# quantumgizmos/ldpc

Measured on AMD Instinct MI355X. Metric: syndromes_per_sec_batched_bp50_product_sum_ldpc36_n10k, higher is better.
Workload: dtype f64; 1 GPU; configs[1]: (3,6)-regular LDPC n=10000 (m=5000, E=30000), product_sum flooding BP, max_iter=50, batch=65536 syndromes per GPU, BSC p=0.09, code seed 1, error seed 7; batch_per_gpu=65536, global_batch=65536, max_iter=50, outputs=decoding u8, log_prob_ratios f64, iterations i32, converge u8, parallelism=single GPU, no process group, device_math=libm_exact

## Files before the change

### include/ldpc_hip.h

```cpp
#ifndef LDPC_HIP_H
#define LDPC_HIP_H

#include <stdint.h>

#ifdef __cplusplus
extern "C" {
#endif

typedef enum {
    LDPC_HIP_OK = 0,
    LDPC_HIP_ERR_INVALID = -1,
    LDPC_HIP_ERR_DEVICE = -2,
    LDPC_HIP_ERR_NOMEM = -3,
    LDPC_HIP_ERR_UNSUPPORTED = -4
} ldpc_hip_status;

#define LDPC_HIP_PRODUCT_SUM 0
#define LDPC_HIP_MINIMUM_SUM 1

typedef struct {
    int32_t m;
    int32_t n;
    int32_t nnz;
    const int32_t *csr_row_ptr;
// ... 79 lines not shown
int ldpc_hip_bp_last_phase_ms(ldpc_hip_bp *h, float *persistent_ms, float *per_pass_ms);

int64_t ldpc_hip_bp_workspace_bytes(const ldpc_hip_bp *h, int64_t batch);

int ldpc_hip_bp_set_tuning(ldpc_hip_bp *h, int32_t waves_per_workgroup, int32_t max_chunk_tiles);

int ldpc_hip_bp_set_ring(ldpc_hip_bp *h, int32_t depth);

int ldpc_hip_bp_set_handoff(ldpc_hip_bp *h, int32_t threshold_tiles);

int ldpc_hip_bp_set_small_code_kernel(ldpc_hip_bp *h, int32_t mode);
int ldpc_hip_bp_set_debug_switch(ldpc_hip_bp *h, const char *name, int32_t value);

#define LDPC_HIP_MATH_LIBM_EXACT 0
#define LDPC_HIP_MATH_FAST 1
int ldpc_hip_bp_set_math(ldpc_hip_bp *h, int32_t math_mode);

int ldpc_hip_bp_clock_probe(ldpc_hip_bp *h, uint64_t *cycles, uint64_t *ticks, double *tick_hz);

int ldpc_hip_bp_copy_probe(ldpc_hip_bp *h, int64_t tiles, int32_t segments_per_tile, int32_t passes, float *ms, double *gbytes_per_s);

int64_t ldpc_hip_debug_device_buf_bytes(void);

void *ldpc_hip_host_alloc(size_t bytes);
void ldpc_hip_host_free(void *p);

const char *ldpc_hip_last_error(void);
const char *ldpc_hip_version(void);

typedef struct ldpc_hip_bp_multi ldpc_hip_bp_multi;
int ldpc_hip_bp_multi_create(const ldpc_hip_bp_desc *desc , const int32_t *device_ids,
                             int32_t ndev, ldpc_hip_bp_multi **out);
void ldpc_hip_bp_multi_destroy(ldpc_hip_bp_multi *mh);
int32_t ldpc_hip_bp_multi_devices(const ldpc_hip_bp_multi *mh);
ldpc_hip_bp *ldpc_hip_bp_multi_handle(ldpc_hip_bp_multi *mh, int32_t i);
int ldpc_hip_bp_multi_decode_batch(ldpc_hip_bp_multi *mh, int32_t with_osd, const uint8_t *syndromes, int64_t batch,
                                   uint8_t *decoding, double *llr, int32_t *iterations, uint8_t *converge);
int ldpc_hip_bp_multi_last_kernel_ms(ldpc_hip_bp_multi *mh, float *ms_per_device);
int ldpc_hip_bp_multi_set_staging(ldpc_hip_bp_multi *mh, int32_t force);

#ifdef __cplusplus
}
#endif
#endif
```

### ldpc_amd/_lib.py

```python
from __future__ import annotations

import ctypes as C
import os

_HERE = os.path.dirname(os.path.abspath(__file__))
LIB_PATH = os.environ.get("LDPC_HIP_LIB") or os.path.join(_HERE, "lib", "libldpc_hip.so")

SYMBOLS = (
    "ldpc_hip_bp_create", "ldpc_hip_bp_destroy", "ldpc_hip_bp_set_channel", "ldpc_hip_bp_set_params",
    "ldpc_hip_bp_set_stream", "ldpc_hip_bp_set_schedule", "ldpc_hip_bp_set_random_serial", "ldpc_hip_bp_get_schedule_order", "ldpc_hip_bp_decode_batch", "ldpc_hip_bp_decode_batch_async", "ldpc_hip_bposd0_decode_batch", "ldpc_hip_bposd0_decode_batch_async",
    "ldpc_hip_bp_set_osd", "ldpc_hip_bposd_get_status", "ldpc_hip_bp_set_osd_kernel", "ldpc_hip_bp_set_repack", "ldpc_hip_bp_set_serial_kernel", "ldpc_hip_bposd_decode_batch", "ldpc_hip_bposd_decode_batch_async",
    "ldpc_hip_bp_set_observables", "ldpc_hip_bp_decode_b8", "ldpc_hip_bp_soft_info_decode_batch", "ldpc_hip_pack_b8", "ldpc_hip_unpack_b8", "ldpc_hip_bp_last_phase_ms", "ldpc_hip_bp_clock_probe", "ldpc_hip_bp_copy_probe", "ldpc_hip_debug_device_buf_bytes", "ldpc_hip_host_alloc", "ldpc_hip_host_free",
    "ldpc_hip_gf2_mulvec_batch", "ldpc_hip_gen_bsc_syndromes", "ldpc_hip_bp_last_kernel_ms",
    "ldpc_hip_bp_workspace_bytes", "ldpc_hip_bp_set_tuning", "ldpc_hip_bp_set_math", "ldpc_hip_bp_set_ring", "ldpc_hip_bp_set_small_code_kernel", "ldpc_hip_bp_set_handoff", "ldpc_hip_last_error", "ldpc_hip_version",
    "ldpc_hip_bp_set_debug_switch", "ldpc_hip_bp_multi_create", "ldpc_hip_bp_multi_destroy", "ldpc_hip_bp_multi_devices", "ldpc_hip_bp_multi_handle",
    "ldpc_hip_bp_multi_decode_batch", "ldpc_hip_bp_multi_last_kernel_ms", "ldpc_hip_bp_multi_set_staging",
    "ldpc_hip_bp_decode_batch_priors", "ldpc_hip_bp_decode_batch_priors_async", "ldpc_hip_bposd0_decode_batch_priors", "ldpc_hip_bposd0_decode_batch_priors_async",
)


class BpDesc(C.Structure):
    _fields_ = [
        ("m", C.c_int32), ("n", C.c_int32), ("nnz", C.c_int32),
        ("csr_row_ptr", C.POINTER(C.c_int32)), ("csr_col_idx", C.POINTER(C.c_int32)),
        ("channel_probs", C.POINTER(C.c_double)),
        ("max_iter", C.c_int32), ("bp_method", C.c_int32),
        ("ms_scaling_factor", C.c_double), ("device", C.c_int32),
    ]


class LdpcHipError(RuntimeError):
    pass


_lib = None
# ... 32 lines not shown
            getattr(lib, name).argtypes = [vp, vp, i64, vp, vp, vp, vp, vp]
    lib.ldpc_hip_bp_set_osd.argtypes = [vp, i32, i32]
    lib.ldpc_hip_bposd_get_status.argtypes = [vp, vp, i64]
    lib.ldpc_hip_bp_set_osd_kernel.argtypes = [vp, i32]
    lib.ldpc_hip_bp_set_repack.argtypes = [vp, i32]
    lib.ldpc_hip_bp_set_serial_kernel.argtypes = [vp, i32]
    lib.ldpc_hip_bp_set_observables.argtypes = [vp, i32, vp, vp]
    lib.ldpc_hip_bp_decode_b8.argtypes = [vp, vp, i64, i32, vp, vp, vp, vp]
    lib.ldpc_hip_pack_b8.argtypes = [vp, vp, i64, i32, vp]
    lib.ldpc_hip_unpack_b8.argtypes = [vp, vp, i64, i32, vp]
    lib.ldpc_hip_bp_soft_info_decode_batch.argtypes = [vp, vp, i64, C.c_double, C.c_double, vp, vp, vp, vp, vp]
    lib.ldpc_hip_bposd_decode_batch.argtypes = [vp, vp, i64, vp, vp, vp, vp]
    lib.ldpc_hip_bposd_decode_batch_async.argtypes = [vp, vp, i64, vp, vp, vp, vp]
    lib.ldpc_hip_gf2_mulvec_batch.argtypes = [vp, vp, i64, vp]
    lib.ldpc_hip_gen_bsc_syndromes.argtypes = [vp, u64, u64, i64, i64, vp, vp]
    lib.ldpc_hip_bp_last_kernel_ms.argtypes = [vp, C.POINTER(C.c_float)]
    lib.ldpc_hip_bp_last_phase_ms.argtypes = [vp, C.POINTER(C.c_float), C.POINTER(C.c_float)]
    lib.ldpc_hip_bp_clock_probe.argtypes = [vp, C.POINTER(u64), C.POINTER(u64), C.POINTER(C.c_double)]
    if not os.environ.get("LDPC_HIP_LIB") or hasattr(lib, "ldpc_hip_bp_copy_probe"):
        lib.ldpc_hip_bp_copy_probe.argtypes = [vp, C.c_int64, C.c_int32, C.c_int32, C.POINTER(C.c_float), C.POINTER(C.c_double)]
    if not os.environ.get("LDPC_HIP_LIB") or hasattr(lib, "ldpc_hip_debug_device_buf_bytes"):
        lib.ldpc_hip_debug_device_buf_bytes.argtypes = []
        lib.ldpc_hip_debug_device_buf_bytes.restype = i64
    lib.ldpc_hip_host_alloc.argtypes = [C.c_size_t]
    lib.ldpc_hip_host_alloc.restype = C.c_void_p
    lib.ldpc_hip_host_free.argtypes = [vp]
    lib.ldpc_hip_host_free.restype = None
    lib.ldpc_hip_bp_workspace_bytes.argtypes = [vp, i64]
    lib.ldpc_hip_bp_workspace_bytes.restype = i64
    lib.ldpc_hip_bp_set_tuning.argtypes = [vp, i32, i32]
    lib.ldpc_hip_bp_set_math.argtypes = [vp, i32]
    lib.ldpc_hip_bp_set_ring.argtypes = [vp, i32]
    lib.ldpc_hip_bp_set_small_code_kernel.argtypes = [vp, i32]
    lib.ldpc_hip_bp_set_debug_switch.argtypes = [vp, C.c_char_p, i32]
    lib.ldpc_hip_bp_set_handoff.argtypes = [vp, i32]
    lib.ldpc_hip_bp_multi_create.argtypes = [C.POINTER(BpDesc), C.POINTER(i32), i32, C.POINTER(vp)]
    lib.ldpc_hip_bp_multi_destroy.argtypes = [vp]
    lib.ldpc_hip_bp_multi_destroy.restype = None
    lib.ldpc_hip_bp_multi_devices.argtypes = [vp]
    lib.ldpc_hip_bp_multi_devices.restype = i32
    lib.ldpc_hip_bp_multi_handle.argtypes = [vp, i32]
    lib.ldpc_hip_bp_multi_handle.restype = vp
    lib.ldpc_hip_bp_multi_decode_batch.argtypes = [vp, i32, vp, i64, vp, vp, vp, vp]
    lib.ldpc_hip_bp_multi_last_kernel_ms.argtypes = [vp, C.POINTER(C.c_float)]
    lib.ldpc_hip_bp_multi_set_staging.argtypes = [vp, i32]
    lib.ldpc_hip_last_error.restype = C.c_char_p
# ... 46 lines not shown
```

### ldpc_amd/csrc/bp_device_common.h

```cpp
#pragma once

#include <hip/hip_runtime.h>
#include <hip/hip_ext.h>

#include <cfloat>
#include <cmath>
#include <cstdarg>
#include <cstdint>
#include <cstdio>
#include <cstring>
#include <string>
#include <vector>
#include <cstddef>

#include "../../include/ldpc_hip.h"
#include "bp_math.h"


#define LDPC_WAVE 64


struct BpArgs {
    int32_t m, n, nnz, max_iter;
    double ms_scaling_factor;
    int64_t batch;
    const int32_t *row_ptr, *col_idx;
    const int32_t *col_ptr, *csc_edge;
    const double *llr0;
    double *A;
    double *C;
    const uint64_t *par;
    const uint64_t *nzm;
    const uint64_t *invalid;
    uint64_t *dec;
    uint64_t *dcur;
    double *llr_t;
    int32_t *iters;
    uint8_t *conv;
    struct TileState *state;
    unsigned *counters;
    int32_t *handoff_list;
    int32_t total_tiles, handoff_threshold;
// ... 370 lines not shown
```

### ldpc_amd/csrc/bp_spread_kernels.h

```cpp
#pragma once

#include "bp_device_common.h"

struct SpreadArgs {
    BpArgs bp;
    int32_t n_tiles;
    int32_t nodes;
    int32_t round;
    unsigned *host_flag;
    unsigned seq;
    int32_t slot0;
    const double *llr0_t;
};

__device__ __forceinline__ int spread_count(const SpreadArgs &a) { return a.n_tiles >= 0 ? a.n_tiles : (int)a.bp.counters[1]; }

__global__ void __launch_bounds__(64) bp_spread_compact_kernel(const SpreadArgs a) {
    const int lane = threadIdx.x;
    const int n_tiles = spread_count(a);
    int kept = 0;
    for (int s0 = 0; s0 < n_tiles; s0 += 64) {
        const int slot = s0 + lane;
        int32_t tile = 0;
        bool live = false;
        if (slot < n_tiles) {
            tile = a.bp.handoff_list[slot];
            live = a.round <= a.bp.state[tile].end_round;
        }
        const uint64_t mask = __ballot(live);
        __builtin_amdgcn_wave_barrier();
        if (live) a.bp.handoff_list[kept + lane_rank(mask)] = tile;
        kept += __builtin_popcountll(mask);
    }
    if (lane == 0) a.bp.counters[1] = (unsigned)kept;
}
// ... 85 lines not shown
                if (k < d) { e[k] = sload(a.bp.csc_edge + cs + k); c[k] = Ct.ld(l8, e[k]); }
            llr = bit_column<METHOD, MATH, DC>(c, e, d, prior, At, l8, !last || a.bp.keep_state != 0);
        } else {
            double temp = prior;
            for (int k = 0; k < d; ++k) {
                const int ee = sload(a.bp.csc_edge + cs + k);
                At.st(l8, ee, temp);
                temp += Ct.ld(l8, ee);
            }
            llr = temp;
            double sfx = 0.0;
            for (int k = d - 1; k >= 0; --k) {
                const int ee = sload(a.bp.csc_edge + cs + k);
                At.st(l8, ee, edge_form<METHOD, MATH>(At.ld(l8, ee) + sfx));
                sfx += Ct.ld(l8, ee);
            }
        }
        const uint64_t hard = __ballot(llr <= 0);
        if (lane == 0) a.bp.dcur[tile * n + j] = hard;
        if ((last || each) && want_llr && lane_live) Lt.st(l8, j, llr);
    }
    } while (LOOP && (slot += (int)gridDim.y) < spread_count(a));
}

template <bool LOOP = false>
__global__ void __launch_bounds__(256) bp_spread_synd_kernel(const SpreadArgs a) {
    int64_t tile;
    const TileState *st;
    int it;
    uint64_t done;
    int slot = a.slot0 + (int)blockIdx.y;
    if (LOOP) { if (slot >= spread_count(a)) return; }
    else if (!spread_tile(a, slot, tile, st, it, done)) return;
    do {
    if (LOOP && !spread_tile(a, slot, tile, st, it, done)) continue;
    const int i = blockIdx.x * blockDim.x + threadIdx.x;
    uint64_t unsat = 0;
    if (i < a.bp.m) {
        const uint64_t *dcur = a.bp.dcur + tile * a.bp.n;
        uint64_t cand = 0;
        for (int e = a.bp.row_ptr[i]; e < a.bp.row_ptr[i + 1]; ++e) cand ^= dcur[a.bp.col_idx[e]];
        unsat = cand ^ a.bp.par[tile * a.bp.m + i];
    }
    unsat = wave_or(unsat);
    if ((threadIdx.x & 63) == 0 && unsat) atomicOr(&a.bp.state[tile].unsat[a.round & 1], (unsigned long long)unsat);
    } while (LOOP && (slot += (int)gridDim.y) < spread_count(a));
// ... 106 lines not shown
```

### ldpc_amd/csrc/host_handle.h

```cpp
#pragma once

#include <algorithm>
#include <array>
#include <chrono>
#include <random>
#include <atomic>
#include <thread>

#include <sys/mman.h>


inline thread_local std::string g_last_error;

static int fail(int code, const char *fmt, ...) {
    char buf[512];
    va_list ap;
    va_start(ap, fmt);
    vsnprintf(buf, sizeof buf, fmt, ap);
    va_end(ap);
    g_last_error = buf;
    return code;
}

#define HIPCHK(expr)                                                                          \
// ... 17 lines not shown
    ~DeviceBuf() { release(); }
    int ensure(size_t bytes) {
        if (bytes <= cap) return 0;
        release();
        hipError_t e = hipMalloc(&p, bytes);
        if (e != hipSuccess) {
            p = nullptr;
            return fail(LDPC_HIP_ERR_NOMEM, "hipMalloc(%zu bytes) failed: %s", bytes,
                        hipGetErrorString(e));
        }
        cap = bytes;
        g_device_buf_bytes += (long long)bytes;
        return 0;
    }
    void release() {
        if (p) (void)hipFree(p);
        g_device_buf_bytes -= (long long)cap;
        p = nullptr;
        cap = 0;
    }
};

static const char *const k_switch_names[] = {"PS_TEAM", "EXPLICIT_INIT", "OSD_UNBLOCKED", "OSD_PLANES",
                                             "PS_TEAM_WAVES", "EDGE_STATIC_PCT", "EDGE_CHUNK", "NO_HOST_PIPELINE", "NO_DIRECT_LLR", "HOST_CHUNK_ROWS", "TIME_SMALL_CALLS", "REL_LDS", "HOST_PIPE_TIMING", "REL_LEVELS", "REL_PROF", "REL_SCRATCH_IN_L", "SER_RING", "SER_WAVES", "SER_LANE_MAX", "SER_LANE_THREADS", "SER_WAVES2", "RESIDENT", "SER_NO_REMAINDER", "SER_ROUND_TILES", "VAR_RING", "VAR_RING_UNITS", "SPREAD_NODES", "SER_VAR", "SER_VAR_UNITS", "REL_EXT", "OSD_COLLECT_AFTER", "EDGE_CLAMP", "OSD_NO_FLAT"};
constexpr int k_n_switches = (int)(sizeof(k_switch_names) / sizeof(k_switch_names[0]));

struct ldpc_hip_bp {
    int32_t switches[k_n_switches];
    int sw(const char *name) const {
        for (int i = 0; i < k_n_switches; ++i)
            if (!std::strcmp(name, k_switch_names[i])) return switches[i];
        return -1;
    }
    bool on(const char *name) const { return sw(name) > 0; }
    int device = 0;
    int32_t m = 0, n = 0, nnz = 0;
    int32_t max_iter = 1, bp_method = 0;
    double ms_scaling_factor = 1.0;
    int32_t max_row_deg = 0, max_col_deg = 0;
    int32_t waves_per_wg = 0;
    int32_t math_mode = LDPC_HIP_MATH_LIBM_EXACT;
    bool regular = false;
    int32_t ring_depth = 2;
    int32_t small_mode = -1;
    std::vector<int32_t> h_row_ptr, h_col_idx;
    std::vector<int32_t> h_col_ptr, h_csc_edge, h_csc_row;
    int wave_dr = 0, wave_dc = 0;
    int wave_ps_dr = 0, wave_ps_dc = 0;
    DeviceBuf wp_rdeg, wp_col, wp_epos;
    DeviceBuf w_rdeg, w_cdeg, w_col, w_apos, w_prior;
    DeviceBuf d_edge0;
    DeviceBuf var_row_items, var_pair_items;
    bool var_items_built = false;
    double *cont_A = nullptr, *cont_C = nullptr;
    int32_t cont_it_start = 0;
    const int32_t *cont_row_map = nullptr;
    const unsigned *cont_rows_dev = nullptr;
    int64_t cont_late_rows = -1;
    int64_t cont_grid_tiles = 0;
    bool keep_state = false;
    int64_t last_chunk_tiles = 0;
    int edge_rounds = 0;
    DeviceBuf e_partner, e_kind, e_scol, e_prior;
    int32_t handoff = -1;
    DeviceBuf tile_state, handoff_list;
    unsigned *h_counters = nullptr;
    unsigned *h_flag = nullptr, *d_flag = nullptr;
    unsigned flag_seq = 0;
    unsigned long long *d_clk = nullptr;
    int32_t schedule = 1;
    std::vector<int32_t> sched_state;
    std::mt19937 sched_rng;
    int32_t sched_seed_raw = 0;
    bool random_serial = false;
    DeviceBuf rel_ord, rel_dbit, sched_orders, sched_order0;
    DeviceBuf sched_lvl_bits, sched_lvl_ptr;
// ... 171 lines not shown
```

### ldpc_amd/csrc/host_setup.h

```cpp
#pragma once

extern "C" {

const char *ldpc_hip_last_error(void) { return g_last_error.c_str(); }
const char *ldpc_hip_version(void) { return "ldpc_hip 0.1 (gfx950)"; }

int ldpc_hip_bp_create(const ldpc_hip_bp_desc *d, ldpc_hip_bp **out) {
    if (!d || !out) return fail(LDPC_HIP_ERR_INVALID, "null descriptor or output");
    *out = nullptr;
    if (d->m < 0 || d->n < 0 || !d->csr_row_ptr || (d->nnz > 0 && !d->csr_col_idx) || !d->channel_probs)
        return fail(LDPC_HIP_ERR_INVALID, "bad matrix description");
    if (d->csr_row_ptr[0] != 0 || d->csr_row_ptr[d->m] != d->nnz)
        return fail(LDPC_HIP_ERR_INVALID, "csr_row_ptr[0] must be 0 and csr_row_ptr[m] == nnz");
    if (d->max_iter < 1) return fail(LDPC_HIP_ERR_INVALID, "max_iter must be >= 1");
    if (d->bp_method != LDPC_HIP_PRODUCT_SUM && d->bp_method != LDPC_HIP_MINIMUM_SUM)
        return fail(LDPC_HIP_ERR_INVALID, "bp_method must be 0 (product_sum) or 1 (minimum_sum)");
    if (d->nnz >= (1 << 23) || d->n >= (1 << 23))
        return fail(LDPC_HIP_ERR_UNSUPPORTED, "matrices with nnz or n >= 2^23 are not supported");
    int32_t max_row = 0;
    for (int i = 0; i < d->m; ++i) {
        const int lo = d->csr_row_ptr[i], hi = d->csr_row_ptr[i + 1];
        if (hi < lo) return fail(LDPC_HIP_ERR_INVALID, "csr_row_ptr not monotone at row %d", i);
        if (hi - lo > max_row) max_row = hi - lo;
        for (int e = lo; e < hi; ++e) {
// ... 50 lines not shown
            _e = hipMemcpy((dst), (src), sizeof(T) * (size_t)(count), hipMemcpyHostToDevice);   \
        if (_e != hipSuccess) {                                                                 \
            ldpc_hip_bp_destroy(h);                                                             \
            return fail(LDPC_HIP_ERR_DEVICE, "device upload failed: %s", hipGetErrorString(_e)); \
        }                                                                                       \
    } while (0)
    ALLOC_COPY(h->d_row_ptr, d->csr_row_ptr, d->m + 1, int32_t);
    ALLOC_COPY(h->d_col_idx, d->csr_col_idx, d->nnz, int32_t);
    ALLOC_COPY(h->d_col_ptr, col_ptr.data(), d->n + 1, int32_t);
    ALLOC_COPY(h->d_csc_edge, csc_edge.data(), d->nnz, int32_t);
    ALLOC_COPY(h->d_csc_row, csc_row.data(), d->nnz, int32_t);
    ALLOC_COPY(h->d_llr0, d->channel_probs, d->n, double);
    ALLOC_COPY(h->d_osd_wt, d->channel_probs, d->n, double);
#undef ALLOC_COPY
    int rc = upload_priors(h);
    if (rc) { ldpc_hip_bp_destroy(h); return rc; }
    h->sched_state.resize((size_t)d->n);
    for (int j = 0; j < d->n; ++j) h->sched_state[(size_t)j] = j;
    h->h_row_ptr.assign(d->csr_row_ptr, d->csr_row_ptr + d->m + 1);
    h->h_col_idx.assign(d->csr_col_idx, d->csr_col_idx + d->nnz);
    h->h_col_ptr = std::move(col_ptr);
    h->h_csc_edge = std::move(csc_edge);
    h->h_csc_row = std::move(csc_row);
    hipError_t e = hipStreamCreateWithFlags(&h->own_stream, hipStreamNonBlocking);
    if (e == hipSuccess) e = hipEventCreate(&h->ev0);
    if (e == hipSuccess) e = hipEventCreate(&h->ev1);
    if (e == hipSuccess) e = hipEventCreate(&h->ev_mid);
    if (e == hipSuccess) e = hipEventCreate(&h->evp0);
    if (e == hipSuccess) e = hipEventCreate(&h->evp1);
    if (e == hipSuccess) e = hipEventCreate(&h->evp_mid);
    if (e == hipSuccess) e = hipEventCreate(&h->ev_hist);
    if (e == hipSuccess) e = hipEventCreateWithFlags(&h->ev_done, hipEventDisableTiming);
    if (e == hipSuccess) e = hipHostMalloc((void **)&h->h_flag, 64, hipHostMallocMapped | hipHostMallocCoherent);
    if (e == hipSuccess) { std::memset(h->h_flag, 0, 64); e = hipHostGetDevicePointer((void **)&h->d_flag, h->h_flag, 0); }
    if (e == hipSuccess) e = hipMalloc((void **)&h->d_clk, 16);
    if (e == hipSuccess) e = hipMemset(h->d_clk, 0, 16);
    if (e != hipSuccess) {
        ldpc_hip_bp_destroy(h);
        return fail(LDPC_HIP_ERR_DEVICE, "stream/event creation failed: %s", hipGetErrorString(e));
    }
    h->stream = h->own_stream;
    *out = h;
    return LDPC_HIP_OK;
}

void ldpc_hip_bp_destroy(ldpc_hip_bp *h) {
// ... 177 lines not shown
    const int64_t tiles = (batch + LDPC_WAVE - 1) / LDPC_WAVE;
    return tiles * (2ll * 8 * h->nnz * LDPC_WAVE + 2ll * 8 * h->m + 8 + 8ll * h->n +
                    8ll * h->n * LDPC_WAVE  + 8ll * h->n * LDPC_WAVE );
}

int ldpc_hip_bp_last_kernel_ms(ldpc_hip_bp *h, float *ms) {
    if (!h || !ms) return fail(LDPC_HIP_ERR_INVALID, "null argument");
    *ms = 0.f;
    if (!h->timed) return LDPC_HIP_OK;
    HIPCHK(hipSetDevice(h->device));
    HIPCHK(hipEventSynchronize(h->ev1));
    float last = 0.f;
    HIPCHK(hipEventElapsedTime(&last, h->ev0, h->ev1));
    *ms = h->accumulated_ms + last;
    if (h->timed_prev) {
        HIPCHK(hipEventElapsedTime(&last, h->evp0, h->evp1));
        *ms += last;
    }
    return LDPC_HIP_OK;
}

int64_t ldpc_hip_debug_device_buf_bytes(void) { return (int64_t)g_device_buf_bytes.load(); }

void *ldpc_hip_host_alloc(size_t bytes) {
    void *p = nullptr;
    if (hipHostMalloc(&p, bytes ? bytes : 1, hipHostMallocDefault) != hipSuccess) {
        (void)hipGetLastError();
        return nullptr;
    }
    return p;
}

void ldpc_hip_host_free(void *p) {
    if (p) (void)hipHostFree(p);
}

int ldpc_hip_bp_clock_probe(ldpc_hip_bp *h, uint64_t *cycles, uint64_t *ticks, double *tick_hz) {
    if (!h || !cycles || !ticks || !tick_hz) return fail(LDPC_HIP_ERR_INVALID, "null argument");
    HIPCHK(hipSetDevice(h->device));
    HIPCHK(hipStreamSynchronize(h->stream));
    unsigned long long v[2] = {0, 0};
    HIPCHK(hipMemcpy(v, h->d_clk, 16, hipMemcpyDeviceToHost));
    int khz = 0;
    HIPCHK(hipDeviceGetAttribute(&khz, hipDeviceAttributeWallClockRate, h->device));
    *cycles = v[0];
    *ticks = v[1];
// ... 56 lines not shown
```

### ldpc_amd/csrc/host_stream.h

```cpp
#pragma once


template <bool LOOP>
static void pick_spread(const ldpc_hip_bp *h, bool nt, spread_kernel_t &kc, spread_kernel_t &kb) {
    with_method_math(h, [&](auto M, auto F) { pick_spread_m<M, F, LOOP>(h->max_row_deg, h->max_col_deg, nt, kc, kb); });
}
static void pick_spread_row_priors(const ldpc_hip_bp *h, bool nt, spread_kernel_t &kc, spread_kernel_t &kb) {
    with_method_math(h, [&](auto M, auto F) { pick_spread_m<M, F, false, true>(h->max_row_deg, h->max_col_deg, nt, kc, kb); });
}

static int ensure_var_ring_items(ldpc_hip_bp *h, int W) {
    if (h->var_items_built) return 0;
    const int m = h->m, n = h->n, pairs = (n + 1) / 2;
    std::vector<int32_t> col_ptr((size_t)n + 1, 0);
    for (int32_t c : h->h_col_idx) ++col_ptr[(size_t)c + 1];
    for (int j = 0; j < n; ++j) col_ptr[(size_t)j + 1] += col_ptr[(size_t)j];
    auto interleave = [W](std::vector<std::array<int32_t, 4>> &items) {
        auto units = [](const std::array<int32_t, 4> &it) { return (it[2] + (it[3] > 0 ? it[3] : 0) + 1) / 2; };
        std::stable_sort(items.begin(), items.end(), [&](const std::array<int32_t, 4> &x, const std::array<int32_t, 4> &y) { return units(x) > units(y); });
        std::vector<std::array<int32_t, 4>> out;
        out.reserve(items.size());
        size_t lo = 0, hi = items.size();
        for (bool heavy = true; lo < hi; heavy = !heavy)
            for (int k = 0; k < W && lo < hi; ++k) out.push_back(heavy ? items[lo++] : items[--hi]);
        items.swap(out);
    };
    std::vector<std::array<int32_t, 4>> rows((size_t)m), prs((size_t)pairs);
    for (int i = 0; i < m; ++i) rows[(size_t)i] = {h->h_row_ptr[(size_t)i], i, h->h_row_ptr[(size_t)i + 1] - h->h_row_ptr[(size_t)i], 0};
    for (int g = 0; g < pairs; ++g) {
        const int j0 = 2 * g, j1 = j0 + 1;
        prs[(size_t)g] = {col_ptr[(size_t)j0], g, col_ptr[(size_t)j0 + 1] - col_ptr[(size_t)j0], j1 < n ? col_ptr[(size_t)j1 + 1] - col_ptr[(size_t)j1] : -1};
// ... 174 lines not shown
                if ((rc = h->d_edge0.ensure(sizeof(double) * (size_t)h->n))) return rc;
                const dim3 ge((unsigned)((h->n + 255) / 256));
                with_method_math(h, [&](auto M, auto F) { hipLaunchKernelGGL((bp_edge0_kernel<M, F>), ge, dim3(256), 0, st, h->d_llr0, h->n, (double *)h->d_edge0.p); });
                a.edge0 = (const double *)h->d_edge0.p;
            }
            hipLaunchKernelGGL(kern.fn, dim3((unsigned)tiles), dim3((unsigned)(waves * LDPC_WAVE)), (unsigned)dyn_lds, st, a);
            HIPCHK(hipGetLastError());
            HIPCHK(hipEventRecord(h->ev_mid, st));
            h->timed_mid = true;
            if (handoff > 0 && h->max_iter > 1) {
                grid_tiles = (unsigned)(tiles < handoff ? tiles : handoff);
                sa.n_tiles = -1;
                sa.nodes = 4;
            }
        }
        if (grid_tiles > 0) {
            spread_kernel_t kc, kb, kcl, kbl;
            const bool nt = (double)grid_tiles * 2.0 * (double)per_tile_msg > 384.0 * 1024.0 * 1024.0;
            pick_spread<false>(h, nt, kc, kb);
            pick_spread<true>(h, nt, kcl, kbl);
            if (rp) pick_spread_row_priors(h, nt, kc, kb);
            const auto k_finish = rp ? bp_spread_finish_kernel<false, true> : bp_spread_finish_kernel<false>;
            const unsigned per_wg = 4u * (unsigned)sa.nodes;
            const dim3 gc((unsigned)(h->m ? (h->m + per_wg - 1) / per_wg : 1), grid_tiles), gb((unsigned)(h->n ? (h->n + per_wg - 1) / per_wg : 1), grid_tiles);
            const dim3 gs((unsigned)(h->m ? (h->m + 255) / 256 : 1), grid_tiles), gf((unsigned)(h->n ? (h->n + 63) / 64 : 1), grid_tiles);
            const int rounds = h->max_iter - (first_round ? first_round : a.it_start);
            const volatile unsigned *flag = h->h_flag;
            const bool may_compact = rows_dev != nullptr && h->cont_late_rows >= 0 && h->cont_late_rows <= 24 && grid_tiles > 40;
            bool compacted = false;
            for (int round = 0; round < rounds; ++round) {
                if (*flag == sa.seq) break;
                sa.round = round;
                sa.slot0 = 0;
                if (may_compact && round >= 8 && round % 8 == 0) {
                    hipLaunchKernelGGL(bp_spread_compact_kernel, dim3(1), dim3(64), 0, st, sa);
                    sa.n_tiles = -1;
                    compacted = true;
                }
                if (!compacted) {
                    hipLaunchKernelGGL(kc, gc, dim3(256), 0, st, sa);
                    hipLaunchKernelGGL(kb, gb, dim3(256), 0, st, sa);
                    hipLaunchKernelGGL(bp_spread_synd_kernel<false>, gs, dim3(256), 0, st, sa);
                    hipLaunchKernelGGL(k_finish, gf, dim3(256), 0, st, sa);
                } else {
                    SpreadArgs sb = sa;
                    sb.slot0 = 32;
                    hipLaunchKernelGGL(kc, dim3(gc.x, 32), dim3(256), 0, st, sa);
                    hipLaunchKernelGGL(kcl, dim3(gc.x, 8), dim3(256), 0, st, sb);
                    hipLaunchKernelGGL(kb, dim3(gb.x, 32), dim3(256), 0, st, sa);
                    hipLaunchKernelGGL(kbl, dim3(gb.x, 8), dim3(256), 0, st, sb);
                    hipLaunchKernelGGL(bp_spread_synd_kernel<false>, dim3(gs.x, 32), dim3(256), 0, st, sa);
                    hipLaunchKernelGGL(bp_spread_synd_kernel<true>, dim3(gs.x, 8), dim3(256), 0, st, sb);
                    hipLaunchKernelGGL(bp_spread_finish_kernel<false>, dim3(gf.x, 32), dim3(256), 0, st, sa);
                    hipLaunchKernelGGL(bp_spread_finish_kernel<true>, dim3(gf.x, 8), dim3(256), 0, st, sb);
                }
            }
            HIPCHK(hipGetLastError());
        }
        HIPCHK(hipEventRecord(h->ev1, st));
        h->timed = true;
        HIPCHK(hipGetLastError());

        if (h->n > 0) {
            dim3 g((unsigned)((h->n + 255) / 256), loop_tiles);
            hipLaunchKernelGGL(unpack_decoding_kernel, g, dim3(256), 0, st,
                               (const uint64_t *)h->dec.p, nb, h->n, decoding + b0 * h->n, row_map, rows_dev);
            if (llr) {
                dim3 gt((unsigned)((h->n + LDPC_WAVE - 1) / LDPC_WAVE), loop_tiles);
                hipLaunchKernelGGL(transpose_llr_kernel, gt, dim3(256), 0, st,
                                   (const double *)h->llr_t.p, nb, h->n, llr + (size_t)b0 * h->n, row_map, rows_dev);
            }
        }
        HIPCHK(hipGetLastError());
// ... 135 lines not shown
```

### ldpc_amd/csrc/tu_stream.hip

```cpp
#include "bp_device_common.h"
#include "bp_stream_kernel.h"
#include "bp_spread_kernels.h"
#include "io_kernels.h"

#include "host_handle.h"

typedef void (*bp_kernel_t)(const BpArgs);
typedef void (*spread_kernel_t)(const SpreadArgs);

template <int METHOD, int MATH, bool LOOP, bool RP = false>
static void pick_spread_m(int max_row, int max_col, bool nt, spread_kernel_t &kc, spread_kernel_t &kb) {
    if (nt) {
        kc = max_row <= 8 ? bp_spread_check_kernel<METHOD, MATH, 8, 1, LOOP> : bp_spread_check_kernel<METHOD, MATH, 16, 1, LOOP>;
        kb = max_col <= 4 ? bp_spread_bit_kernel<METHOD, MATH, 4, 1, LOOP, RP> : bp_spread_bit_kernel<METHOD, MATH, 8, 1, LOOP, RP>;
    } else {
        kc = max_row <= 8 ? bp_spread_check_kernel<METHOD, MATH, 8, 0, LOOP> : bp_spread_check_kernel<METHOD, MATH, 16, 0, LOOP>;
        kb = max_col <= 4 ? bp_spread_bit_kernel<METHOD, MATH, 4, 0, LOOP, RP> : bp_spread_bit_kernel<METHOD, MATH, 8, 0, LOOP, RP>;
    }
}

struct KernelChoice {
    bp_kernel_t fn;
    int ring_slot_bytes;
    int ring_depth;
    int max_waves = 16;
    bool var_ring = false;
};

template <int METHOD, int MATH>
static KernelChoice pick_kernel(int max_row, int max_col, int ring_depth, bool var_ring) {
    if (var_ring) return {bp_decode_kernel<METHOD, MATH, 16, 8, LDPC_RING_VAR>, 0, 0, stream_max_waves(16, LDPC_RING_VAR), true};
    if (ring_depth == 2 && max_row == 6 && max_col == 3) return {bp_decode_kernel<METHOD, MATH, 6, 3, 2>, 3 * 1024, 2};
    if (ring_depth >= 3 && max_row == 6 && max_col == 3) return {bp_decode_kernel<METHOD, MATH, 6, 3, 3>, 3 * 1024, 3};
    if (ring_depth >= (METHOD == LDPC_HIP_PRODUCT_SUM ? 3 : 2) && max_row == 8 && max_col == 4) return {bp_decode_kernel<METHOD, MATH, 8, 4, 3>, 4 * 1024, 3};
    if (METHOD == LDPC_HIP_PRODUCT_SUM && ring_depth >= 2 && max_row == 4 && max_col == 3) return {bp_decode_kernel<METHOD, MATH, 4, 3, 2>, 3 * 1024, 2};
    if (METHOD == LDPC_HIP_PRODUCT_SUM && ring_depth >= 2 && max_row == 5 && max_col == 3) return {bp_decode_kernel<METHOD, MATH, 5, 3, 2>, 3 * 1024, 2};
    if (max_row <= 4 && max_col <= 3) return {bp_decode_kernel<METHOD, MATH, 4, 3, 0>, 0, 0};
    if (max_row <= 6 && max_col <= 3) return {bp_decode_kernel<METHOD, MATH, 6, 3, 0>, 0, 0};
    if (max_row <= 8 && max_col <= 4) return {bp_decode_kernel<METHOD, MATH, 8, 4, 0>, 0, 0, stream_max_waves(8, 0)};
    if (max_row <= 8 && max_col <= 8) return {bp_decode_kernel<METHOD, MATH, 8, 8, 0>, 0, 0, stream_max_waves(8, 0)};
// ... 6 lines not shown
```

Baseline: 105,200 syndromes/s.

## Add degree-class-sorted spread kernels with exact compile-time degrees

Nodes are bucketed by degree on the host into padded 64-node units, and new check and bit spread kernels are added. Each workgroup looks up its degree class and runs a loop with the degree fixed at compile time instead of a runtime-degree loop. The aim is to remove the branching and masked work of the generic max-degree kernels and allow full unrolling with registers. The cost is extra order-array loads, padding units, and more kernel instantiations. It is enabled by default on the spread path, and a SPREAD_GENERIC switch restores the old kernels.

```diff
diff --git a/include/ldpc_hip.h b/include/ldpc_hip.h
--- a/include/ldpc_hip.h
+++ b/include/ldpc_hip.h
@@ -125,6 +125,8 @@
 
 int64_t ldpc_hip_debug_device_buf_bytes(void);
 
+int64_t ldpc_hip_debug_degree_classes(const int32_t *ptr, int32_t count, int32_t lo, int32_t hi, int32_t *order, int64_t order_cap, int32_t *bounds);
+
 void *ldpc_hip_host_alloc(size_t bytes);
 void ldpc_hip_host_free(void *p);
 
diff --git a/ldpc_amd/_lib.py b/ldpc_amd/_lib.py
--- a/ldpc_amd/_lib.py
+++ b/ldpc_amd/_lib.py
@@ -10,7 +10,7 @@
     "ldpc_hip_bp_create", "ldpc_hip_bp_destroy", "ldpc_hip_bp_set_channel", "ldpc_hip_bp_set_params",
     "ldpc_hip_bp_set_stream", "ldpc_hip_bp_set_schedule", "ldpc_hip_bp_set_random_serial", "ldpc_hip_bp_get_schedule_order", "ldpc_hip_bp_decode_batch", "ldpc_hip_bp_decode_batch_async", "ldpc_hip_bposd0_decode_batch", "ldpc_hip_bposd0_decode_batch_async",
     "ldpc_hip_bp_set_osd", "ldpc_hip_bposd_get_status", "ldpc_hip_bp_set_osd_kernel", "ldpc_hip_bp_set_repack", "ldpc_hip_bp_set_serial_kernel", "ldpc_hip_bposd_decode_batch", "ldpc_hip_bposd_decode_batch_async",
-    "ldpc_hip_bp_set_observables", "ldpc_hip_bp_decode_b8", "ldpc_hip_bp_soft_info_decode_batch", "ldpc_hip_pack_b8", "ldpc_hip_unpack_b8", "ldpc_hip_bp_last_phase_ms", "ldpc_hip_bp_clock_probe", "ldpc_hip_bp_copy_probe", "ldpc_hip_debug_device_buf_bytes", "ldpc_hip_host_alloc", "ldpc_hip_host_free",
+    "ldpc_hip_bp_set_observables", "ldpc_hip_bp_decode_b8", "ldpc_hip_bp_soft_info_decode_batch", "ldpc_hip_pack_b8", "ldpc_hip_unpack_b8", "ldpc_hip_bp_last_phase_ms", "ldpc_hip_bp_clock_probe", "ldpc_hip_bp_copy_probe", "ldpc_hip_debug_device_buf_bytes", "ldpc_hip_debug_degree_classes", "ldpc_hip_host_alloc", "ldpc_hip_host_free",
     "ldpc_hip_gf2_mulvec_batch", "ldpc_hip_gen_bsc_syndromes", "ldpc_hip_bp_last_kernel_ms",
     "ldpc_hip_bp_workspace_bytes", "ldpc_hip_bp_set_tuning", "ldpc_hip_bp_set_math", "ldpc_hip_bp_set_ring", "ldpc_hip_bp_set_small_code_kernel", "ldpc_hip_bp_set_handoff", "ldpc_hip_last_error", "ldpc_hip_version",
     "ldpc_hip_bp_set_debug_switch", "ldpc_hip_bp_multi_create", "ldpc_hip_bp_multi_destroy", "ldpc_hip_bp_multi_devices", "ldpc_hip_bp_multi_handle",
@@ -89,6 +89,9 @@
     if not os.environ.get("LDPC_HIP_LIB") or hasattr(lib, "ldpc_hip_debug_device_buf_bytes"):
         lib.ldpc_hip_debug_device_buf_bytes.argtypes = []
         lib.ldpc_hip_debug_device_buf_bytes.restype = i64
+    if not os.environ.get("LDPC_HIP_LIB") or hasattr(lib, "ldpc_hip_debug_degree_classes"):
+        lib.ldpc_hip_debug_degree_classes.argtypes = [vp, i32, i32, i32, vp, i64, vp]
+        lib.ldpc_hip_debug_degree_classes.restype = i64
     lib.ldpc_hip_host_alloc.argtypes = [C.c_size_t]
     lib.ldpc_hip_host_alloc.restype = C.c_void_p
     lib.ldpc_hip_host_free.argtypes = [vp]
diff --git a/ldpc_amd/csrc/bp_device_common.h b/ldpc_amd/csrc/bp_device_common.h
--- a/ldpc_amd/csrc/bp_device_common.h
+++ b/ldpc_amd/csrc/bp_device_common.h
@@ -18,6 +18,14 @@
 
 
 #define LDPC_WAVE 64
+
+#define LDPC_SPREAD_UNIT 64
+#define LDPC_ROW_CLASS_LO 2
+#define LDPC_ROW_CLASS_HI 16
+#define LDPC_COL_CLASS_LO 1
+#define LDPC_COL_CLASS_HI 8
+#define LDPC_ROW_CLASSES (LDPC_ROW_CLASS_HI - LDPC_ROW_CLASS_LO + 2)
+#define LDPC_COL_CLASSES (LDPC_COL_CLASS_HI - LDPC_COL_CLASS_LO + 2)
 
 
 struct BpArgs {
diff --git a/ldpc_amd/csrc/bp_spread_kernels.h b/ldpc_amd/csrc/bp_spread_kernels.h
--- a/ldpc_amd/csrc/bp_spread_kernels.h
+++ b/ldpc_amd/csrc/bp_spread_kernels.h
@@ -11,6 +11,8 @@
     unsigned seq;
     int32_t slot0;
     const double *llr0_t;
+    const int32_t *row_order, *col_order;
+    int32_t row_bounds[LDPC_ROW_CLASSES + 1], col_bounds[LDPC_COL_CLASSES + 1];
 };
 
 __device__ __forceinline__ int spread_count(const SpreadArgs &a) { return a.n_tiles >= 0 ? a.n_tiles : (int)a.bp.counters[1]; }
@@ -142,6 +144,160 @@
     }
     } while (LOOP && (slot += (int)gridDim.y) < spread_count(a));
 }
+
+template <int NCLS>
+__device__ __forceinline__ int spread_class(const int32_t (&bounds)[NCLS + 1], int per_wg) {
+    const int unit = (int)(blockIdx.x * (unsigned)per_wg) / LDPC_SPREAD_UNIT;
+    if (unit >= bounds[NCLS]) return -1;
+    int c = 0;
+#pragma unroll
+    for (int q = 1; q < NCLS; ++q) c += unit >= bounds[q] ? 1 : 0;
+    return c;
+}
+
+template <int METHOD, int MATH, int D, class BUF>
+__device__ __forceinline__ void spread_check_rows(const SpreadArgs &a, int64_t tile, int p0, const BUF &At, const BUF &Ct, int lane, int l8,
+                                                  double alpha, const double *log_tab, uint64_t live, double *near_buf) {
+    for (int p = p0; p < p0 + a.nodes; ++p) {
+        const int i = sload(a.row_order + p);
+        if (i < 0) break;
+        const int rs = sload(a.bp.row_ptr + i);
+        const bool neg = (sload(a.bp.nzm + tile * a.bp.m + i) >> lane) & 1ull;
+        const int parity = (int)((sload(a.bp.par + tile * a.bp.m + i) >> lane) & 1ull);
+        double cur[D];
+#pragma unroll
+        for (int k = 0; k < D; ++k) cur[k] = At.ld(l8, rs + k);
+        check_row_live<METHOD, MATH, D>(cur, D, rs, neg, parity, alpha, Ct, l8, log_tab, live, near_buf);
+    }
+}
+
+#define LDPC_ROW_CASE(D) \
+    case (D) - LDPC_ROW_CLASS_LO: \
+        if constexpr ((D) <= DR) spread_check_rows<METHOD, MATH, (D)>(a, tile, p0, At, Ct, lane, l8, alpha, log_tab, ~done, near_bufs[wave]); \
+        break;
+
+template <int METHOD, int MATH, int DR, int NT>
+__global__ void __launch_bounds__(256) bp_spread_check_exact_kernel(const SpreadArgs a) {
+    typedef MsgBufT<NT ? 2 : 0> Buf;
+    __shared__ __attribute__((aligned(16))) double log_tab[256];
+    __shared__ double near_bufs[4][LDPC_NEAR_SLOTS];
+    int64_t tile;
+    const TileState *st;
+    int it;
+    uint64_t done;
+    if (!spread_tile(a, a.slot0 + (int)blockIdx.y, tile, st, it, done)) return;
+    const int cls = spread_class<LDPC_ROW_CLASSES>(a.row_bounds, 4 * a.nodes);
+    if (cls < 0) return;
+    if (METHOD == LDPC_HIP_PRODUCT_SUM && MATH == 0)
+        for (int q = threadIdx.x; q < 256; q += blockDim.x) log_tab[q] = ldpc_math::k_log_tab[q];
+    __syncthreads();
+    const int lane = threadIdx.x & 63;
+    const int wave = __builtin_amdgcn_readfirstlane((int)(threadIdx.x >> 6));
+    const int nnz = a.bp.nnz, l8 = lane * 8;
+    const Buf At = make_msgbuf<Buf>(a.bp.A + (size_t)tile * (size_t)nnz * LDPC_WAVE, (unsigned)nnz);
+    const Buf Ct = make_msgbuf<Buf>(a.bp.C + (size_t)tile * (size_t)nnz * LDPC_WAVE, (unsigned)nnz);
+    const double alpha = (a.bp.ms_scaling_factor == 0.0) ? 1.0 - ldexp(1.0, -it) : a.bp.ms_scaling_factor;
+    const int p0 = (blockIdx.x * 4 + wave) * a.nodes;
+    switch (cls) {
+        LDPC_ROW_CASE(2) LDPC_ROW_CASE(3) LDPC_ROW_CASE(4) LDPC_ROW_CASE(5) LDPC_ROW_CASE(6) LDPC_ROW_CASE(7) LDPC_ROW_CASE(8) LDPC_ROW_CASE(9)
+        LDPC_ROW_CASE(10) LDPC_ROW_CASE(11) LDPC_ROW_CASE(12) LDPC_ROW_CASE(13) LDPC_ROW_CASE(14) LDPC_ROW_CASE(15) LDPC_ROW_CASE(16)
+        default:
+            for (int p = p0; p < p0 + a.nodes; ++p) {
+                const int i = sload(a.row_order + p);
+                if (i < 0) break;
+                const int rs = sload(a.bp.row_ptr + i), d = sload(a.bp.row_ptr + i + 1) - rs;
+                const bool neg = (sload(a.bp.nzm + tile * a.bp.m + i) >> lane) & 1ull;
+                const int parity = (int)((sload(a.bp.par + tile * a.bp.m + i) >> lane) & 1ull);
+                if (d == 1) {
+                    const double cur[1] = {At.ld(l8, rs)};
+                    check_row<METHOD, MATH, 1>(cur, 1, rs, neg, parity, alpha, Ct, l8, log_tab);
+                } else if (d > 1) {
+                    check_row_streamed<METHOD, MATH>(d, rs, neg, parity, alpha, At, Ct, l8, log_tab);
+                }
+            }
+            break;
+    }
+}
+#undef LDPC_ROW_CASE
+
+template <int METHOD, int MATH, int D, bool RP, class BUF>
+__device__ __forceinline__ void spread_bit_columns(const SpreadArgs &a, int64_t tile, int p0, const BUF &At, const BUF &Ct, const BUF &Lt, const BUF &Pt,
+                                                   int lane, int l8, bool messages, bool store_llr) {
+    for (int p = p0; p < p0 + a.nodes; ++p) {
+        const int j = sload(a.col_order + p);
+        if (j < 0) break;
+        const int cs = sload(a.bp.col_ptr + j);
+        const double prior = RP ? Pt.ld(l8, j) : sload(a.bp.llr0 + j);
+        int e[D];
+        double c[D];
+#pragma unroll
+        for (int k = 0; k < D; ++k) e[k] = sload(a.bp.csc_edge + cs + k);
+#pragma unroll
+        for (int k = 0; k < D; ++k) c[k] = Ct.ld(l8, e[k]);
+        const double llr = bit_column<METHOD, MATH, D>(c, e, D, prior, At, l8, messages);
+        const uint64_t hard = __ballot(llr <= 0);
+        if (lane == 0) a.bp.dcur[tile * a.bp.n + j] = hard;
+        if (store_llr) Lt.st(l8, j, llr);
+    }
+}
+
+#define LDPC_COL_CASE(D) \
+    case (D) - LDPC_COL_CLASS_LO: \
+        if constexpr ((D) <= DC) spread_bit_columns<METHOD, MATH, (D), RP>(a, tile, p0, At, Ct, Lt, Pt, lane, l8, messages, store_llr); \
+        break;
+
+template <int METHOD, int MATH, int DC, int NT, bool RP = false>
+__global__ void __launch_bounds__(256) bp_spread_bit_exact_kernel(const SpreadArgs a) {
+    typedef MsgBufT<NT ? 2 : 0> Buf;
+    int64_t tile;
+    const TileState *st;
+    int it;
+    uint64_t done;
+    if (!spread_tile(a, a.slot0 + (int)blockIdx.y, tile, st, it, done)) return;
+    const int cls = spread_class<LDPC_COL_CLASSES>(a.col_bounds, 4 * a.nodes);
+    if (cls < 0) return;
+    const int lane = threadIdx.x & 63;
+    const int wave = __builtin_amdgcn_readfirstlane((int)(threadIdx.x >> 6));
+    const int nnz = a.bp.nnz, n = a.bp.n, l8 = lane * 8;
+    const Buf At = make_msgbuf<Buf>(a.bp.A + (size_t)tile * (size_t)nnz * LDPC_WAVE, (unsigned)nnz);
+    const Buf Ct = make_msgbuf<Buf>(a.bp.C + (size_t)tile * (size_t)nnz * LDPC_WAVE, (unsigned)nnz);
+    const bool want_llr = a.bp.llr_t != nullptr;
+    const Buf Lt = make_msgbuf<Buf>(want_llr ? a.bp.llr_t + (size_t)tile * (size_t)n * LDPC_WAVE : a.bp.A, want_llr ? (unsigned)n : 0u);
+    const Buf Pt = make_msgbuf<Buf>(RP ? const_cast<double *>(a.llr0_t) + (size_t)tile * (size_t)n * LDPC_WAVE : a.bp.A, RP ? (unsigned)n : 0u);
+    const bool last = it == a.bp.max_iter;
+    const bool lane_live = !((done >> lane) & 1ull);
+    const bool each = st->llr_each[a.round & 1] != 0;
+    const bool messages = !last || a.bp.keep_state != 0;
+    const bool store_llr = (last || each) && want_llr && lane_live;
+    const int p0 = (blockIdx.x * 4 + wave) * a.nodes;
+    switch (cls) {
+        LDPC_COL_CASE(1) LDPC_COL_CASE(2) LDPC_COL_CASE(3) LDPC_COL_CASE(4) LDPC_COL_CASE(5) LDPC_COL_CASE(6) LDPC_COL_CASE(7) LDPC_COL_CASE(8)
+        default:
+            for (int p = p0; p < p0 + a.nodes; ++p) {
+                const int j = sload(a.col_order + p);
+                if (j < 0) break;
+                const int cs = sload(a.bp.col_ptr + j), d = sload(a.bp.col_ptr + j + 1) - cs;
+                double temp = RP ? Pt.ld(l8, j) : sload(a.bp.llr0 + j);
+                for (int k = 0; k < d; ++k) {
+                    const int ee = sload(a.bp.csc_edge + cs + k);
+                    At.st(l8, ee, temp);
+                    temp += Ct.ld(l8, ee);
+                }
+                const double llr = temp;
+                double sfx = 0.0;
+                for (int k = d - 1; k >= 0; --k) {
+                    const int ee = sload(a.bp.csc_edge + cs + k);
+                    At.st(l8, ee, edge_form<METHOD, MATH>(At.ld(l8, ee) + sfx));
+                    sfx += Ct.ld(l8, ee);
+                }
+                const uint64_t hard = __ballot(llr <= 0);
+                if (lane == 0) a.bp.dcur[tile * n + j] = hard;
+                if (store_llr) Lt.st(l8, j, llr);
+            }
+            break;
+    }
+}
+#undef LDPC_COL_CASE
 
 template <bool LOOP = false>
 __global__ void __launch_bounds__(256) bp_spread_synd_kernel(const SpreadArgs a) {
diff --git a/ldpc_amd/csrc/host_handle.h b/ldpc_amd/csrc/host_handle.h
--- a/ldpc_amd/csrc/host_handle.h
+++ b/ldpc_amd/csrc/host_handle.h
@@ -63,8 +63,26 @@
 };
 
 static const char *const k_switch_names[] = {"PS_TEAM", "EXPLICIT_INIT", "OSD_UNBLOCKED", "OSD_PLANES",
-                                             "PS_TEAM_WAVES", "EDGE_STATIC_PCT", "EDGE_CHUNK", "NO_HOST_PIPELINE", "NO_DIRECT_LLR", "HOST_CHUNK_ROWS", "TIME_SMALL_CALLS", "REL_LDS", "HOST_PIPE_TIMING", "REL_LEVELS", "REL_PROF", "REL_SCRATCH_IN_L", "SER_RING", "SER_WAVES", "SER_LANE_MAX", "SER_LANE_THREADS", "SER_WAVES2", "RESIDENT", "SER_NO_REMAINDER", "SER_ROUND_TILES", "VAR_RING", "VAR_RING_UNITS", "SPREAD_NODES", "SER_VAR", "SER_VAR_UNITS", "REL_EXT", "OSD_COLLECT_AFTER", "EDGE_CLAMP", "OSD_NO_FLAT"};
+                                             "PS_TEAM_WAVES", "EDGE_STATIC_PCT", "EDGE_CHUNK", "NO_HOST_PIPELINE", "NO_DIRECT_LLR", "HOST_CHUNK_ROWS", "TIME_SMALL_CALLS", "REL_LDS", "HOST_PIPE_TIMING", "REL_LEVELS", "REL_PROF", "REL_SCRATCH_IN_L", "SER_RING", "SER_WAVES", "SER_LANE_MAX", "SER_LANE_THREADS", "SER_WAVES2", "RESIDENT", "SER_NO_REMAINDER", "SER_ROUND_TILES", "VAR_RING", "VAR_RING_UNITS", "SPREAD_NODES", "SER_VAR", "SER_VAR_UNITS", "REL_EXT", "OSD_COLLECT_AFTER", "EDGE_CLAMP", "OSD_NO_FLAT", "SPREAD_GENERIC"};
 constexpr int k_n_switches = (int)(sizeof(k_switch_names) / sizeof(k_switch_names[0]));
+
+struct DegreeClasses {
+    std::vector<int32_t> order, bounds;
+};
+static DegreeClasses build_degree_classes(const int32_t *ptr, int count, int lo, int hi) {
+    const int ncls = hi - lo + 2;
+    auto cls_of = [&](int node) { const int d = ptr[node + 1] - ptr[node]; return d >= lo && d <= hi ? d - lo : ncls - 1; };
+    std::vector<int32_t> members((size_t)ncls, 0);
+    for (int v = 0; v < count; ++v) ++members[(size_t)cls_of(v)];
+    DegreeClasses dc;
+    dc.bounds.assign((size_t)ncls + 1, 0);
+    for (int c = 0; c < ncls; ++c) dc.bounds[(size_t)c + 1] = dc.bounds[(size_t)c] + (members[(size_t)c] + LDPC_SPREAD_UNIT - 1) / LDPC_SPREAD_UNIT;
+    dc.order.assign((size_t)dc.bounds[(size_t)ncls] * LDPC_SPREAD_UNIT, -1);
+    std::vector<size_t> fill((size_t)ncls);
+    for (int c = 0; c < ncls; ++c) fill[(size_t)c] = (size_t)dc.bounds[(size_t)c] * LDPC_SPREAD_UNIT;
+    for (int v = 0; v < count; ++v) dc.order[fill[(size_t)cls_of(v)]++] = v;
+    return dc;
+}
 
 struct ldpc_hip_bp {
     int32_t switches[k_n_switches];
@@ -93,6 +111,8 @@
     DeviceBuf d_edge0;
     DeviceBuf var_row_items, var_pair_items;
     bool var_items_built = false;
+    DeviceBuf spread_row_order, spread_col_order;
+    std::vector<int32_t> spread_row_bounds, spread_col_bounds;
     double *cont_A = nullptr, *cont_C = nullptr;
     int32_t cont_it_start = 0;
     const int32_t *cont_row_map = nullptr;
diff --git a/ldpc_amd/csrc/host_setup.h b/ldpc_amd/csrc/host_setup.h
--- a/ldpc_amd/csrc/host_setup.h
+++ b/ldpc_amd/csrc/host_setup.h
@@ -96,6 +96,19 @@
     h->h_col_ptr = std::move(col_ptr);
     h->h_csc_edge = std::move(csc_edge);
     h->h_csc_row = std::move(csc_row);
+    {
+        DegreeClasses rows = build_degree_classes(h->h_row_ptr.data(), d->m, LDPC_ROW_CLASS_LO, LDPC_ROW_CLASS_HI);
+        DegreeClasses cols = build_degree_classes(h->h_col_ptr.data(), d->n, LDPC_COL_CLASS_LO, LDPC_COL_CLASS_HI);
+        hipError_t ue = hipSuccess;
+        if (!rows.order.empty() && (rc = h->spread_row_order.ensure(sizeof(int32_t) * rows.order.size())) == 0)
+            ue = hipMemcpy(h->spread_row_order.p, rows.order.data(), sizeof(int32_t) * rows.order.size(), hipMemcpyHostToDevice);
+        if (rc == 0 && ue == hipSuccess && !cols.order.empty() && (rc = h->spread_col_order.ensure(sizeof(int32_t) * cols.order.size())) == 0)
+            ue = hipMemcpy(h->spread_col_order.p, cols.order.data(), sizeof(int32_t) * cols.order.size(), hipMemcpyHostToDevice);
+        if (rc) { ldpc_hip_bp_destroy(h); return rc; }
+        if (ue != hipSuccess) { ldpc_hip_bp_destroy(h); return fail(LDPC_HIP_ERR_DEVICE, "device upload failed: %s", hipGetErrorString(ue)); }
+        h->spread_row_bounds = std::move(rows.bounds);
+        h->spread_col_bounds = std::move(cols.bounds);
+    }
     hipError_t e = hipStreamCreateWithFlags(&h->own_stream, hipStreamNonBlocking);
     if (e == hipSuccess) e = hipEventCreate(&h->ev0);
     if (e == hipSuccess) e = hipEventCreate(&h->ev1);
@@ -319,6 +332,14 @@
 
 int64_t ldpc_hip_debug_device_buf_bytes(void) { return (int64_t)g_device_buf_bytes.load(); }
 
+int64_t ldpc_hip_debug_degree_classes(const int32_t *ptr, int32_t count, int32_t lo, int32_t hi, int32_t *order, int64_t order_cap, int32_t *bounds) {
+    if (!ptr || count < 0 || lo < 0 || hi < lo || !bounds || (order_cap > 0 && !order)) { fail(LDPC_HIP_ERR_INVALID, "degree classes: bad arguments"); return -1; }
+    const DegreeClasses dc = build_degree_classes(ptr, count, lo, hi);
+    std::copy(dc.bounds.begin(), dc.bounds.end(), bounds);
+    if ((int64_t)dc.order.size() <= order_cap) std::copy(dc.order.begin(), dc.order.end(), order);
+    return (int64_t)dc.order.size();
+}
+
 void *ldpc_hip_host_alloc(size_t bytes) {
     void *p = nullptr;
     if (hipHostMalloc(&p, bytes ? bytes : 1, hipHostMallocDefault) != hipSuccess) {
diff --git a/ldpc_amd/csrc/host_stream.h b/ldpc_amd/csrc/host_stream.h
--- a/ldpc_amd/csrc/host_stream.h
+++ b/ldpc_amd/csrc/host_stream.h
@@ -7,6 +7,13 @@
 }
 static void pick_spread_row_priors(const ldpc_hip_bp *h, bool nt, spread_kernel_t &kc, spread_kernel_t &kb) {
     with_method_math(h, [&](auto M, auto F) { pick_spread_m<M, F, false, true>(h->max_row_deg, h->max_col_deg, nt, kc, kb); });
+}
+
+static void pick_spread_exact(const ldpc_hip_bp *h, bool nt, bool rp, spread_kernel_t &kc, spread_kernel_t &kb) {
+    with_method_math(h, [&](auto M, auto F) {
+        if (rp) pick_spread_exact_m<M, F, true>(h->max_row_deg, h->max_col_deg, nt, kc, kb);
+        else pick_spread_exact_m<M, F>(h->max_row_deg, h->max_col_deg, nt, kc, kb);
+    });
 }
 
 static int ensure_var_ring_items(ldpc_hip_bp *h, int W) {
@@ -227,7 +234,17 @@
             if (rp) pick_spread_row_priors(h, nt, kc, kb);
             const auto k_finish = rp ? bp_spread_finish_kernel<false, true> : bp_spread_finish_kernel<false>;
             const unsigned per_wg = 4u * (unsigned)sa.nodes;
-            const dim3 gc((unsigned)(h->m ? (h->m + per_wg - 1) / per_wg : 1), grid_tiles), gb((unsigned)(h->n ? (h->n + per_wg - 1) / per_wg : 1), grid_tiles);
+            const dim3 gcl((unsigned)(h->m ? (h->m + per_wg - 1) / per_wg : 1), grid_tiles), gbl((unsigned)(h->n ? (h->n + per_wg - 1) / per_wg : 1), grid_tiles);
+            dim3 gc = gcl, gb = gbl;
+            if (h->sw("SPREAD_GENERIC") == 0 && h->m > 0 && h->n > 0 && LDPC_SPREAD_UNIT % per_wg == 0) {
+                pick_spread_exact(h, nt, rp, kc, kb);
+                sa.row_order = (const int32_t *)h->spread_row_order.p;
+                sa.col_order = (const int32_t *)h->spread_col_order.p;
+                std::copy(h->spread_row_bounds.begin(), h->spread_row_bounds.end(), sa.row_bounds);
+                std::copy(h->spread_col_bounds.begin(), h->spread_col_bounds.end(), sa.col_bounds);
+                gc.x = (unsigned)sa.row_bounds[LDPC_ROW_CLASSES] * (LDPC_SPREAD_UNIT / per_wg);
+                gb.x = (unsigned)sa.col_bounds[LDPC_COL_CLASSES] * (LDPC_SPREAD_UNIT / per_wg);
+            }
             const dim3 gs((unsigned)(h->m ? (h->m + 255) / 256 : 1), grid_tiles), gf((unsigned)(h->n ? (h->n + 63) / 64 : 1), grid_tiles);
             const int rounds = h->max_iter - (first_round ? first_round : a.it_start);
             const volatile unsigned *flag = h->h_flag;
@@ -251,9 +268,9 @@
                     SpreadArgs sb = sa;
                     sb.slot0 = 32;
                     hipLaunchKernelGGL(kc, dim3(gc.x, 32), dim3(256), 0, st, sa);
-                    hipLaunchKernelGGL(kcl, dim3(gc.x, 8), dim3(256), 0, st, sb);
+                    hipLaunchKernelGGL(kcl, dim3(gcl.x, 8), dim3(256), 0, st, sb);
                     hipLaunchKernelGGL(kb, dim3(gb.x, 32), dim3(256), 0, st, sa);
-                    hipLaunchKernelGGL(kbl, dim3(gb.x, 8), dim3(256), 0, st, sb);
+                    hipLaunchKernelGGL(kbl, dim3(gbl.x, 8), dim3(256), 0, st, sb);
                     hipLaunchKernelGGL(bp_spread_synd_kernel<false>, dim3(gs.x, 32), dim3(256), 0, st, sa);
                     hipLaunchKernelGGL(bp_spread_synd_kernel<true>, dim3(gs.x, 8), dim3(256), 0, st, sb);
                     hipLaunchKernelGGL(bp_spread_finish_kernel<false>, dim3(gf.x, 32), dim3(256), 0, st, sa);
diff --git a/ldpc_amd/csrc/tu_stream.hip b/ldpc_amd/csrc/tu_stream.hip
--- a/ldpc_amd/csrc/tu_stream.hip
+++ b/ldpc_amd/csrc/tu_stream.hip
@@ -16,6 +16,17 @@
     } else {
         kc = max_row <= 8 ? bp_spread_check_kernel<METHOD, MATH, 8, 0, LOOP> : bp_spread_check_kernel<METHOD, MATH, 16, 0, LOOP>;
         kb = max_col <= 4 ? bp_spread_bit_kernel<METHOD, MATH, 4, 0, LOOP, RP> : bp_spread_bit_kernel<METHOD, MATH, 8, 0, LOOP, RP>;
+    }
+}
+
+template <int METHOD, int MATH, bool RP = false>
+static void pick_spread_exact_m(int max_row, int max_col, bool nt, spread_kernel_t &kc, spread_kernel_t &kb) {
+    if (nt) {
+        kc = max_row <= 8 ? bp_spread_check_exact_kernel<METHOD, MATH, 8, 1> : bp_spread_check_exact_kernel<METHOD, MATH, 16, 1>;
+        kb = max_col <= 4 ? bp_spread_bit_exact_kernel<METHOD, MATH, 4, 1, RP> : bp_spread_bit_exact_kernel<METHOD, MATH, 8, 1, RP>;
+    } else {
+        kc = max_row <= 8 ? bp_spread_check_exact_kernel<METHOD, MATH, 8, 0> : bp_spread_check_exact_kernel<METHOD, MATH, 16, 0>;
+        kb = max_col <= 4 ? bp_spread_bit_exact_kernel<METHOD, MATH, 4, 0, RP> : bp_spread_bit_exact_kernel<METHOD, MATH, 8, 0, RP>;
     }
 }
 
```

Measured after the change: 103,900 syndromes/s. 0.988x the previous value.
